# Nesquiko/Latticeum

Hardware: AMD Instinct MI355X
Metric: fold-steps/sec (Ajtai commit+fold) at d=1024 (higher is better)
Workload: dtype u64 (Goldilocks mod-p integer); 1 GPU; configs[2] at d=1024: commit+fold step, X^1024+1, W=16384, kappa=32, K=15; rho is an input; transcript, linearization, sumchecks, Mz outside the step; d=1024, W=16384, N=81920, kappa=32

## Files before the change

include/lf.h:

```cpp
#ifndef LATTICEUM_AMD_LF_H
#define LATTICEUM_AMD_LF_H
#include <stddef.h>
#include <stdint.h>

#ifdef __cplusplus
extern "C" {
#endif

typedef struct lf_ctx lf_ctx;
typedef struct lf_ajtai lf_ajtai;
typedef struct lf_transcript lf_transcript;
typedef struct lf_comm lf_comm;
typedef struct lf_ccs lf_ccs;

enum lf_status {
  LF_OK = 0,
  LF_ERR_INVALID_ARG = 1,
  LF_ERR_UNSUPPORTED_RING = 2,
  LF_ERR_WRONG_WITNESS_LENGTH = 3,
  LF_ERR_WRONG_COMMITMENT_LENGTH = 4,
  LF_ERR_WRONG_AJTAI_DIMENSIONS = 5,
  LF_ERR_DECOMPOSITION_OVERFLOW = 6,
  LF_ERR_INCORRECT_LENGTH = 7,
  LF_ERR_CHALLENGE_BYTES = 8,
// ... 147 lines not shown
int lf_dev_fold_step_sharded(lf_ctx *ctx, const lf_ajtai *aj, const lf_params *pr, size_t W,
                             const lf_fold_step_bufs *b, lf_comm *comm);

int lf_comm_unique_id(uint8_t *id, size_t len);
int lf_comm_init(lf_ctx *ctx, int nranks, int rank, const uint8_t *id, size_t len, lf_comm **out);
int lf_comm_wrap(lf_ctx *ctx, void *nccl_comm, lf_comm **out);
void lf_comm_destroy(lf_comm *comm);
int lf_comm_size(const lf_comm *comm);
int lf_comm_rank(const lf_comm *comm);
int lf_comm_allreduce_modp(lf_ctx *ctx, lf_comm *comm, uint64_t *x, size_t n);
int lf_fold_reduce_allranks(lf_ctx *ctx, lf_comm *comm, uint64_t *cm0, size_t cm0_len, uint64_t *f0,
                            size_t f0_len);

int lf_dev_fold_lcccs(lf_ctx *ctx, int d, int nwit, const uint64_t *rho, const uint64_t *rho_coeff,
                      const uint64_t *eta, size_t t, const uint64_t *xwh, size_t l1, const uint64_t *theta,
                      uint64_t *u0, uint64_t *x0, uint64_t *v0);
int lf_dev_compute_x_s(lf_ctx *ctx, const lf_params *pr, const uint64_t *x, size_t m, uint64_t *x_s);

int lf_dev_poseidon2_permute(lf_ctx *ctx, uint64_t *states, size_t n);
int lf_dev_poseidon2_permute_rounds(lf_ctx *ctx, uint64_t *states, size_t n, int rounds);
int lf_dev_gl_probe(lf_ctx *ctx, int op, const uint64_t *a, const uint64_t *b, int s, int m, uint64_t *out,
                    size_t n);
int lf_ctx_fold_flag(lf_ctx *ctx, int *out);
enum { LF_PLAN_FOLDING = 0, LF_PLAN_LIN = 1, LF_PLAN_LIN_EQ = 2 };
int lf_sumcheck_round_plan(int d, size_t half, int nf, int kind, int out[8]);
int lf_sumcheck_dot_plan(int d, size_t n, int out[4]);
int lf_dev_fill_uniform(lf_ctx *ctx, uint64_t *out, size_t n, uint64_t seed);
int lf_dev_modp_sum(lf_ctx *ctx, const uint64_t *in, int nparts, size_t len, uint64_t *out);

int lf_dev_limb_split(lf_ctx *ctx, const uint64_t *x, size_t n, uint64_t *lo, uint64_t *hi);
int lf_dev_limb_join(lf_ctx *ctx, const uint64_t *lo, const uint64_t *hi, size_t n, uint64_t *out);

enum { LF_COMB_FOLDING = 0, LF_COMB_LINEARIZATION = 1 };
typedef struct {
  int kind;
  int nk, tau, bsmall;
  const uint64_t *mu;
  int q;
  const uint64_t *c;
  const int *S_off;
  const int *S_idx;
} lf_comb;
int lf_dev_eq_table(lf_ctx *ctx, int d, const uint64_t *r, int nv, uint64_t *out);
int lf_dev_get_fhat(lf_ctx *ctx, int d, const uint64_t *f_coeff, size_t N, int nv, uint64_t *out);
int lf_dev_mle_fix_first(lf_ctx *ctx, int d, const uint64_t *in, size_t in_stride, int nm, int nv,
                         const uint64_t *r_base, uint64_t *out, size_t out_stride);
// ... 307 lines not shown
```

latticeum_amd/__init__.py:

```python
from __future__ import annotations

import ctypes as C
from dataclasses import dataclass

import numpy as np

from ._lib import LfComb, LfFoldStepBufs, LfParams, load

P = (1 << 64) - (1 << 32) + 1
REPR_CANONICAL = 0
REPR_MONTGOMERY = 1
SUPPORTED_D = (24, 16, 32, 64, 128, 256, 512, 1024, 2048, 4096)
AJTAI_SEED_POSEIDON2 = 1
AJTAI_SEED_SPLITMIX = 2


class LfError(RuntimeError):
    def __init__(self, code: int, msg: str):
        super().__init__(f"lf error {code}: {msg}")
        self.code = code


def goldilocks_dp(d: int = 24) -> LfParams:
    return load().lf_goldilocks_dp(d)
# ... 59 lines not shown
            self.lib.lf_stream_destroy(st)
        self._masked = []

    def __del__(self):
        try:
            self.close()
        except Exception:
            pass

    def check(self, rc: int):
        if rc != 0:
            msg = self.lib.lf_ctx_last_error(self.h).decode() or self.lib.lf_status_string(rc).decode()
            raise LfError(rc, msg)

    def set_stream(self, hip_stream: int | None):
        self.check(self.lib.lf_ctx_set_stream(self.h, hip_stream))

    def sync(self):
        self.check(self.lib.lf_ctx_sync(self.h))

    def fold_flag(self) -> int:
        out = C.c_int()
        self.check(self.lib.lf_ctx_fold_flag(self.h, C.byref(out)))
        return out.value

    def use_cu_mask(self, cus):
        cus = list(cus)
        st = self.cu_mask_stream(cus)
        self.set_stream(st)
        self.check(self.lib.lf_ctx_set_cu_count(self.h, len(set(cus))))
        return st

    def set_contract_stream(self, hip_stream: int | None):
        self.check(self.lib.lf_ctx_set_contract_stream(self.h, hip_stream))

    def cu_mask_stream(self, cus):
        cus = list(cus)
        words = (max(cus) // 32 + 1) if cus else 1
        mask = (C.c_uint32 * words)()
        for i in cus:
            mask[i // 32] |= 1 << (i % 32)
        st = C.c_void_p()
        rc = self.lib.lf_stream_create_cu_mask(self.device, mask, words, C.byref(st))
        if rc != 0:
            raise LfError(rc, "lf_stream_create_cu_mask")
        self._masked = getattr(self, "_masked", []) + [st.value]
# ... 1162 lines not shown
```

latticeum_amd/_lib.py:

```python
from __future__ import annotations

import ctypes as C
import os
from pathlib import Path

PKG = Path(__file__).resolve().parent
LIB_PATH = PKG / "liblatticeum_amd.so"

SZ, I, U64, VP = C.c_size_t, C.c_int, C.c_uint64, C.c_void_p
U64P = C.POINTER(C.c_uint64)
U8P = C.POINTER(C.c_uint8)


class LfParams(C.Structure):
    _fields_ = [("d", I), ("B", U64), ("L", I), ("b_small", U64), ("K", I)]


class LfFoldStepBufs(C.Structure):
    _fields_ = [
        ("w_ccs", VP), ("acc_cm", VP), ("acc_f_coeff", VP), ("rho", VP),
        ("f_coeff", VP), ("f", VP), ("cm", VP),
        ("fk_coeff", VP * 2), ("fk", VP * 2), ("wk", VP * 2), ("y", VP * 2),
        ("f0", VP), ("f0_coeff", VP), ("w_ccs0", VP), ("cm0", VP), ("planes", VP * 2),
    ]
# ... 93 lines not shown
    "lf_decompose_witness": (I, [VP, C.POINTER(LfParams), VP, SZ, VP, VP, VP, I]),
    "lf_commit": (I, [VP, VP, C.POINTER(LfParams), VP, SZ, SZ, VP, VP, VP, I]),
    "lf_fold_hot": (I, [VP, VP, C.POINTER(LfParams), VP, VP, VP, VP, SZ, VP, VP, VP, VP, VP, VP, I]),
    "lf_short_challenge": (I, [VP, SZ, I, VP]),
    "lf_poseidon2_permute": (I, [VP, VP, SZ]),
    "lf_dev_crt": (I, [VP, VP, SZ, I]),
    "lf_dev_icrt": (I, [VP, VP, SZ, I]),
    "lf_dev_ring_mul": (I, [VP, VP, VP, VP, SZ, I]),
    "lf_dev_to_montgomery": (I, [VP, VP, SZ]),
    "lf_dev_from_montgomery": (I, [VP, VP, SZ]),
    "lf_dev_witness_from_w_ccs": (I, [VP, C.POINTER(LfParams), VP, SZ, VP, VP]),
    "lf_dev_witness_from_f": (I, [VP, C.POINTER(LfParams), VP, SZ, VP, VP]),
    "lf_dev_witness_from_f_coeff": (I, [VP, C.POINTER(LfParams), VP, SZ, VP, VP]),
    "lf_dev_decompose_witness": (I, [VP, C.POINTER(LfParams), VP, SZ, VP, VP, VP]),
    "lf_dev_ajtai_commit": (I, [VP, VP, C.POINTER(VP), I, VP]),
    "lf_dev_commit_y0": (I, [VP, C.POINTER(LfParams), VP, VP, SZ]),
    "lf_dev_fold": (I, [VP, I, VP, C.POINTER(VP), I, SZ, VP]),
    "lf_dev_fold_step": (I, [VP, VP, C.POINTER(LfParams), SZ, C.POINTER(LfFoldStepBufs)]),
    "lf_dev_fold_step_batch": (I, [VP, I, VP, C.POINTER(LfParams), SZ, VP]),
    "lf_dev_poseidon2_permute": (I, [VP, VP, SZ]),
    "lf_dev_poseidon2_permute_rounds": (I, [VP, VP, SZ, I]),
    "lf_dev_gl_probe": (I, [VP, I, VP, VP, I, I, VP, SZ]),
    "lf_ctx_fold_flag": (I, [VP, C.POINTER(I)]),
    "lf_sumcheck_round_plan": (I, [I, SZ, I, I, C.POINTER(I * 8)]),
    "lf_sumcheck_dot_plan": (I, [I, SZ, C.POINTER(I * 4)]),
    "lf_dev_fhat_lincomb_digits": (I, [VP, I, VP, SZ, SZ, I, I, VP, VP]),
    "lf_dev_fill_uniform": (I, [VP, VP, SZ, U64]),
    "lf_dev_modp_sum": (I, [VP, VP, I, SZ, VP]),
    "lf_dev_limb_split": (I, [VP, VP, SZ, VP, VP]),
    "lf_dev_limb_join": (I, [VP, VP, VP, SZ, VP]),
    "lf_transcript_new": (VP, []),
    "lf_transcript_free": (None, [VP]),
    "lf_transcript_observe": (None, [VP, U64]),
    "lf_transcript_sample": (U64, [VP]),
    "lf_transcript_absorb_ring": (None, [VP, VP, SZ, I, I]),
    "lf_transcript_get_challenge": (None, [VP, VP]),
    "lf_transcript_squeeze_bytes": (None, [VP, VP, SZ]),
    "lf_transcript_get_short_challenges": (I, [VP, I, SZ, VP]),
    "lf_hash_iter": (None, [VP, SZ, VP]),
    "lf_hash_iter_nperm": (SZ, [SZ]),
    "lf_hash_iter_states": (I, [VP, SZ, VP, VP, SZ]),
    "lf_acc_comm": (I, [C.POINTER(LfLcccs), I, VP]),
    "lf_ivc_step_comm": (I, [U64, VP, VP, VP, VP, VP]),
    "lf_state_i_comm": (I, [VP, U64, VP, VP, VP, VP]),
    "lf_vm_regs_comm": (I, [VP, SZ, VP]),
    "lf_vm_mem_ops_vec_comm": (I, [VP, U64, C.c_uint32, C.c_uint32, VP]),
# ... 149 lines not shown
```

latticeum_amd/csrc/api_internal.hpp:

```cpp
#pragma once
#include <hip/hip_runtime.h>
#include <rccl/rccl.h>

#include <cstring>
#include <map>
#include <string>
#include <vector>

#include "../../include/lf.h"
#include "gl.hpp"
#include "kernels.hpp"
#include "launch.hpp"

struct Tables {
  uint64_t *mem = nullptr;
  ring::NegaTables fwd{}, inv{};
};

struct TimedLaunch {
  hipEvent_t a, b;
  int nvec;
  int count = 1;
};

// ... 16 lines not shown

struct lf_ctx {
  int device = 0;
  hipStream_t own = nullptr, cur = nullptr;
  int *d_err = nullptr;
  int *d_sync = nullptr;
  std::string last_error;
  std::map<int, Tables> tables;
  uint64_t *scratch = nullptr;
  size_t scratch_elems = 0;
  uint64_t *ybuf = nullptr;
  size_t ybuf_elems = 0;
  uint4 *frag = nullptr;
  size_t frag_elems = 0;
  uint32_t *smg = nullptr;
  size_t smg_elems = 0;
  uint32_t *fkeys = nullptr;
  size_t fkeys_elems = 0;
  uint64_t *faux = nullptr;
  int32_t *fpart = nullptr;
  size_t fpart_elems = 0;
  size_t faux_elems = 0;
  long fold_flag_at = -1;
  uint64_t *sink = nullptr;
  uint8_t *dead = nullptr;
  size_t dead_elems = 0;
  uint4 *zero80 = nullptr;
  uint32_t *toptbl = nullptr;
  StepState step{};
  int ncu = 0;
  uint64_t *stage = nullptr;
  size_t stage_elems = 0;
  uint64_t *limb = nullptr;
  size_t limb_elems = 0;
  uint64_t *tmp = nullptr;
  size_t tmp_elems = 0;
  uint64_t *sc = nullptr;
  size_t sc_elems = 0;
  uint64_t *ptrs = nullptr;
  size_t ptrs_elems = 0;
  int *sel = nullptr;
  size_t sel_elems = 0;
  uint64_t *rel = nullptr;
  size_t rel_elems = 0;
  uint64_t *hmsg = nullptr;
  size_t hmsg_elems = 0;
// ... 181 lines not shown
```

latticeum_amd/csrc/api_step.hip:

```cpp
#include <algorithm>

#include "api_internal.hpp"

namespace {

struct PhaseTimer {
  lf_ctx *c;
  int phase;
  hipEvent_t a = nullptr;
  PhaseTimer(lf_ctx *ctx, int ph) : c(ctx), phase(ph) {
    if (c->timing && hipEventCreate(&a) == hipSuccess) (void)hipEventRecord(a, c->cur);
  }
  ~PhaseTimer() {
    hipEvent_t b = nullptr;
    if (a && hipEventCreate(&b) == hipSuccess) {
      (void)hipEventRecord(b, c->cur);
      c->pending.push_back({a, b, -1 - phase});
    }
  }
};

bool n4k_ok(const Tables *t, int d, int lbs, int K) { return d == 4096 && lbs == 1 && K <= 15 && t->fwd.tw4; }

enum class Decomp { Plain, Fused1024, Fused24, Fused4k, FusedPow2 };
// ... 229 lines not shown
  if (c->timing) c->pending.push_back({ea, eb, nvec});
  return LF_OK;
}

lfk::OutPtrs fold_dst(const lf_params *pr, const lf_fold_step_bufs *b, size_t kd, uint64_t *commit_cm,
                      bool z0 = false) {
  lfk::OutPtrs dst{};
  const int extra = commit_cm ? 1 : 0;
  if (commit_cm) dst.p[0] = z0 ? b->y[1] : commit_cm;
  for (int s = 0; s < 2; s++)
    for (int k = 1; k < pr->K; k++) dst.p[extra + s * (pr->K - 1) + k - 1] = b->y[s] + (size_t)k * kd;
  return dst;
}

int fold_finish(lf_ctx *c, const lf_ajtai *aj, const lf_params *pr, int lb, int lbs, size_t W,
                const lf_fold_step_bufs *b, uint64_t *cm_i, bool cm1_out = false) {
  const int d = pr->d, L = pr->L, K = pr->K, nw = 2 * K;
  const size_t N = W * (size_t)L, kappa = aj->kappa;
  Tables *t;
  LF_TRY(get_tables(c, d, t));
  LF_HIP(c, lfk::y0_cm0(b->acc_cm, cm_i, b->y[0], b->y[1], b->rho, kappa, d, lbs, K, b->cm0, c->cur, cm1_out));
  const StepState &st = c->step;
  c->fold_flag_at = -1;
  auto fk_rows = [&] {
    lfk::VecPtrs fx{};
    for (int s = 0; s < 2; s++)
      for (int k = 0; k < K; k++) fx.p[s * K + k] = b->fk[s] + (size_t)k * N * d;
    return fx;
  };
  switch (st.N == N ? st.path : FoldPath::Ntt) {
    case FoldPath::Coeff1024:
    case FoldPath::Coeff1024Rows: {
      const size_t tab_u64 = ((size_t)nw * lfk::FOLD_RT + 7) / 8, aux = (size_t)nw * 1024 + tab_u64 + 1;
      LF_TRY(grow(c, c->fkeys, c->fkeys_elems, 2 * N * (size_t)K * 64 + 2 * N));
      uint32_t *nz = c->fkeys + 2 * N * (size_t)K * 64;
      LF_TRY(grow(c, c->faux, c->faux_elems, aux));
      uint64_t *rc = c->faux;
      uint8_t *tab = reinterpret_cast<uint8_t *>(c->faux + (size_t)nw * 1024);
      int *bad = reinterpret_cast<int *>(c->faux + aux - 1);
      c->fold_flag_at = (long)(aux - 1);
      {
        PhaseTimer pt(c, LF_PHASE_FOLD);
        for (int s = 0; s < 2; s++)
          LF_HIP(c, lfk::fold_keys(st.smg_side[s], N, K, c->fkeys + (size_t)s * N * K * 64, c->cur, nz + (size_t)s * N));
        LF_HIP(c, lfk::fold_rho_tables(b->rho, nw, rc, tab, bad, t->inv, c->d_sync, c->cur));
        const int ks_n = lfk::fold_coeff_splits(N, K, c->ncu);
        if (ks_n > 1) LF_TRY(grow(c, c->fpart, c->fpart_elems, (size_t)ks_n * N * 1024));
        const bool in_launch = st.path == FoldPath::Coeff1024Rows;
        const lfk::FoldFallback fb{c->frag, aj->geom.nch, aj->geom.Lp, aj->geom.Wp, st.fold_rows, b->rho, b->f0};
        LF_HIP(c, lfk::fold_coeff(c->fkeys, tab, bad, N, K, b->f0_coeff, c->ncu, c->cur,
                                  ks_n > 1 ? c->fpart : nullptr, in_launch ? &fb : nullptr, L, nz));
        if (!in_launch) LF_HIP(c, lfk::fold(b->rho, fk_rows(), nw, N, d, b->f0, c->cur, bad));
      }
      PhaseTimer pt(c, LF_PHASE_FROM_F);
      LF_HIP(c, lfk::from_fcoeff_n32(b->f0_coeff, W, lb, L, b->f0, b->w_ccs0, t->fwd, bad, c->cur, &t->inv));
      return LF_OK;
    }
    case FoldPath::Masks24:
    case FoldPath::Masks24Packed: {
      const uint2 *m0 = st.masks24[0], *m1 = st.masks24[1];
      LF_TRY(grow(c, c->faux, c->faux_elems, (size_t)nw * 13 + 1));
      uint32_t *rc = reinterpret_cast<uint32_t *>(c->faux);
      int *bad = reinterpret_cast<int *>(c->faux + (size_t)nw * 13);
      c->fold_flag_at = (long)nw * 13;
      {
        PhaseTimer pt(c, LF_PHASE_FOLD);
        LF_HIP(c, lfk::fold_phi72_rho(b->rho, nw, rc, bad, c->cur));
        LF_HIP(c, lfk::fold_phi72_coeff(m0, m1, rc, bad, N, K, L, lb, b->f0_coeff, b->f0, b->w_ccs0, c->cur));
        if (st.path == FoldPath::Masks24Packed)
          LF_HIP(c, lfk::fold_phi72_masks(m0, m1, b->rho, K, N, b->f0, bad, c->cur));
        else
          LF_HIP(c, lfk::fold(b->rho, fk_rows(), nw, N, d, b->f0, c->cur, bad));
      }
      PhaseTimer pt(c, LF_PHASE_FROM_F);
// ... 356 lines not shown
```

latticeum_amd/csrc/fold_coeff.hip:

```cpp
#include "digitpack.hpp"
#include "digits.hpp"
#include "frag.hpp"
#include "kernels.hpp"
#include "launch.hpp"
#include "ntt32.hpp"

namespace lfk {

namespace {
constexpr int FD = 1024;
constexpr int FC_KEYROW = 64;

__device__ __forceinline__ uint32_t spread8(uint32_t x) {
  x &= 0xFFu;
  x = (x | (x << 12)) & 0x000F000Fu;
  x = (x | (x << 6)) & 0x03030303u;
  x = (x | (x << 3)) & 0x11111111u;
  return x;
}

__global__ void __launch_bounds__(256) k_pack_keys(const uint32_t *smg, size_t ncol, int K, uint32_t *keys,
                                                   uint32_t *nz) {
  const size_t t = blockIdx.x * (size_t)blockDim.x + threadIdx.x;
  if (t >= (ncol * 16 + 63) / 64 * 64) return;
// ... 40 lines not shown
      lo[4 * qd + i] = L;
      hi[4 * qd + i] = H;
    }
  uint4 *dst = reinterpret_cast<uint4 *>(keys + col * K * FC_KEYROW + 32 * h + q0);
  for (int k = 0; k < K; k++) {
    uint32_t o[4];
#pragma unroll
    for (int qd = 0; qd < 4; qd++) {
      uint32_t x = 0;
#pragma unroll
      for (int i = 0; i < 4; i++) {
        const int u = 4 * qd + i;
        const uint32_t nib = (k < 8 ? lo[u] >> (4 * k) : hi[u] >> (4 * (k - 8))) & 0xFu;
        x |= (nib | ((hi[u] >> 28) << 4)) << (8 * i);
      }
      o[qd] = x;
    }
    dst[k * (FC_KEYROW / 4)] = make_uint4(o[0], o[1], o[2], o[3]);
  }
}

constexpr int RP_WAVES = 2;
__global__ void __launch_bounds__(64 * RP_WAVES) k_rho_prep(const uint64_t *rho, int nw, uint64_t *rc, uint8_t *tab,
                                                           int *bad, const uint64_t *mid_ig, int *sync) {
  __shared__ uint64_t lds_all[RP_WAVES * n32::WAVE_U64];
  __shared__ uint64_t mid[n32::MID_U64];
  __shared__ int any;
  n32::stage_mid(mid, mid_ig);
  if (threadIdx.x == 0) any = 0;
  __syncthreads();
  const int lane = threadIdx.x & 63, wib = threadIdx.x >> 6, r = lane & 31, h = lane >> 5;
  uint64_t *T = lds_all + wib * n32::WAVE_U64 + h * n32::HALF_U64;
  bool out = false;
  for (int i0 = 2 * RP_WAVES * blockIdx.x; i0 < nw; i0 += 2 * RP_WAVES * gridDim.x) {
    const int i = i0 + 2 * wib + h;
    const bool ok = i < nw;
    uint64_t v[32];
    n32::load_row32(rho + (size_t)(ok ? i : 0) * FD + r, v);
    n32::inverse(v, mid, T, r);
    if (ok) {
      uint64_t *rci = rc + (size_t)i * FD + r;
      uint8_t *ti = tab + (size_t)i * FOLD_RT;
#pragma unroll
      for (int k = 0; k < 32; k++) {
        const int c = r + 32 * k;
        const int64_t sv = signed_rep(v[k]);
        out |= sv > 127 || sv < -127;
        rci[32 * k] = v[k];
        ti[1024 - c] = (uint8_t)(int8_t)sv;
        if (c > 0) ti[2048 - c] = (uint8_t)(int8_t)(-sv);
      }
      for (int o = 2048 + r; o < FOLD_RT; o += 32) ti[o] = 0;
      if (r == 0) ti[0] = 0;
    }
  }
  if (out) any = 1;
  __syncthreads();
  if (threadIdx.x == 0) {
    if (any) atomicOr(&sync[0], 1);
    __threadfence();
    if (atomicAdd(&sync[1], 1) == (int)gridDim.x - 1) {
      *bad = atomicExch(&sync[0], 0);
      atomicExch(&sync[1], 0);
    }
  }
}

__device__ __forceinline__ v4i tile_a(const uint8_t *ri, int o, int sh) {
  const uint32_t *p = reinterpret_cast<const uint32_t *>(ri + (o & ~3));
  const uint32_t d0 = p[0], d1 = p[1], d2 = p[2], d3 = p[3], d4 = p[4];
  v4i a;
  a[0] = (int)__builtin_amdgcn_alignbyte(d1, d0, sh);
  a[1] = (int)__builtin_amdgcn_alignbyte(d2, d1, sh);
  a[2] = (int)__builtin_amdgcn_alignbyte(d3, d2, sh);
  a[3] = (int)__builtin_amdgcn_alignbyte(d4, d3, sh);
  return a;
}

constexpr int FC_MAXW = 30;
__global__ void __launch_bounds__(256, 2) k_fold_coeff(const uint32_t *keys, const uint8_t *tab_g, const int *bad,
                                                      size_t N, int K, uint64_t *f0c, int ks_n, int32_t *part,
                                                      FoldFallback fb, int L, const uint32_t *nz) {
  __shared__ __attribute__((aligned(16))) uint8_t rt[FC_MAXW * FOLD_RT];
  __shared__ uint32_t lut[256];
  static_assert(FC_MAXW * FOLD_RT >= 512 * 9 * 8, "fold_frag_block's LDS fits the rho tables'");
  if (*bad) {
    if (fb.frag) {
      const size_t nvb = (size_t)(FD / 16) * fb.nch;
      for (size_t vb = blockIdx.x; vb < nvb; vb += gridDim.x)
        fold_frag_block(vb, fb.frag, fb.nch, fb.Lp, fb.Wp, fb.fr, fb.rho, FD, N, fb.f0,
                        reinterpret_cast<uint64_t *>(rt));
    }
    return;
  }
  const int nw = 2 * K, tid = threadIdx.x;
  for (int x = tid; x < nw * FOLD_RT / 16; x += blockDim.x)
    reinterpret_cast<uint4 *>(rt)[x] = reinterpret_cast<const uint4 *>(tab_g)[x];
  {
    const uint32_t m = tid & 15, s = tid >> 4;
    uint32_t v = 0;
#pragma unroll
    for (int i = 0; i < 4; i++)
      if ((m >> i) & 1) v |= ((s >> i) & 1 ? 0xFFu : 0x01u) << (8 * i);
    lut[tid] = v;
  }
  __syncthreads();
  const int lane = tid & 63, wv = tid >> 6, col = lane & 31, h = lane >> 5;
  const int sh = (-col) & 3;
  const int obase = 1024 + 16 * h - col;
  const size_t W = N / L, ntl = (W + 31) / 32, ntile = ntl * L;
  for (size_t task = blockIdx.x; task < ntile * ks_n; task += gridDim.x) {
    const size_t tile = task / ks_n;
    const int ks = (int)(task % ks_n), iq0 = 4 * (ks * nw / ks_n), iq1 = 4 * ((ks + 1) * nw / ks_n);
    const size_t grp = (tile % ntl) * 32 + col;
    const bool valid = grp < W;
    const size_t e = grp * L + tile / ntl, ee = valid ? e : 0;
    uint32_t live = nz ? (valid ? nz[ee] | (nz[N + ee] << K) : 0u) : 0xFFFFFFFFu;
// ... 52 lines not shown
    }
    if (valid && ks_n > 1) {
      int32_t *out = part + ((size_t)ks * N + e) * FD + 256 * wv + 4 * h;
#pragma unroll
      for (int tt = 0; tt < 8; tt++)
#pragma unroll
        for (int g = 0; g < 4; g++)
          *reinterpret_cast<v4i *>(out + 32 * tt + 8 * g) =
              (v4i){acc[tt][4 * g], acc[tt][4 * g + 1], acc[tt][4 * g + 2], acc[tt][4 * g + 3]};
    } else if (valid) {
      uint64_t *out = f0c + e * FD + 256 * wv + 4 * h;
      auto fe = [](int x) { return x < 0 ? (uint64_t)(int64_t)x + gl::P : (uint64_t)x; };
#pragma unroll
      for (int tt = 0; tt < 8; tt++)
#pragma unroll
        for (int g = 0; g < 4; g++) {
          ulonglong2 *o = reinterpret_cast<ulonglong2 *>(out + 32 * tt + 8 * g);
          o[0] = make_ulonglong2(fe(acc[tt][4 * g]), fe(acc[tt][4 * g + 1]));
          o[1] = make_ulonglong2(fe(acc[tt][4 * g + 2]), fe(acc[tt][4 * g + 3]));
        }
    }
  }
}
__global__ void k_fold_coeff_sum(const int32_t *part, int ks_n, size_t n, const int *bad, uint64_t *f0c) {
  if (*bad) return;
  const size_t q = blockIdx.x * (size_t)blockDim.x + threadIdx.x;
  if (q >= n / 4) return;
  v4i s = *reinterpret_cast<const v4i *>(part + 4 * q);
  for (int k = 1; k < ks_n; k++) s += *reinterpret_cast<const v4i *>(part + (size_t)k * n + 4 * q);
  auto fe = [](int x) { return x < 0 ? (uint64_t)(int64_t)x + gl::P : (uint64_t)x; };
  ulonglong2 *o = reinterpret_cast<ulonglong2 *>(f0c + 4 * q);
  o[0] = make_ulonglong2(fe(s[0]), fe(s[1]));
  o[1] = make_ulonglong2(fe(s[2]), fe(s[3]));
}
}

int fold_coeff_splits(size_t N, int K, int ncu) {
  const size_t ntile = (N + 31) / 32, cap = 2 * (size_t)ncu;
  int best = 1;
  for (int ks = 2; ks <= 2 * K; ks++)
    if ((2 * K) % ks == 0 && ntile * ks <= cap) best = ks;
  return best;
}

hipError_t fold_keys(const uint32_t *smg, size_t ncol, int K, uint32_t *keys, hipStream_t st, uint32_t *nz) {
  if (K < 1 || K > 15) return hipErrorInvalidValue;
  if (!ncol) return hipSuccess;
  hipLaunchKernelGGL(k_pack_keys, dim3(blocks(ncol * 16, 256)), dim3(256), 0, st, smg, ncol, K, keys,
                     nz);
  return hipGetLastError();
}

hipError_t fold_rho_tables(const uint64_t *rho, int nw, uint64_t *rc, uint8_t *tab, int *bad,
                           const ring::NegaTables &inv, int *sync, hipStream_t st) {
  if (nw < 1 || nw > FC_MAXW || !inv.mid || !sync) return hipErrorInvalidValue;
  const int per = 2 * RP_WAVES;
  hipLaunchKernelGGL(k_rho_prep, dim3((nw + per - 1) / per), dim3(64 * RP_WAVES), 0, st, rho, nw, rc, tab, bad,
                     inv.mid, sync);
  return hipGetLastError();
}

hipError_t fold_coeff(const uint32_t *keys, const uint8_t *tab, const int *bad, size_t N, int K, uint64_t *f0c,
                      int ncu, hipStream_t st, int32_t *part, const FoldFallback *fb, int L, const uint32_t *nz) {
  FoldFallback fbv{};
  if (fb) fbv = *fb;
  if (K < 1 || 2 * K > FC_MAXW || ncu < 1 || L < 1 || N % L) return hipErrorInvalidValue;
  if (!N) return hipSuccess;
  const int ks_n = part ? fold_coeff_splits(N, K, ncu) : 1;
  const size_t ntile = (N / L + 31) / 32 * L;
  const size_t ntask = ntile * ks_n, cap = 2 * (size_t)ncu;
  hipLaunchKernelGGL(k_fold_coeff, dim3((unsigned)(ntask < cap ? ntask : cap)), dim3(256), 0, st, keys, tab, bad, N,
                     K, f0c, ks_n, part, fbv, L, nz);
  if (ks_n > 1) {
    const size_t n = N * FD;
    hipLaunchKernelGGL(k_fold_coeff_sum, dim3(blocks(n / 4, 256)), dim3(256), 0, st, part, ks_n, n, bad,
                       f0c);
  }
  return hipGetLastError();
}

}
```

latticeum_amd/csrc/kernels.hpp:

```cpp
#pragma once
#include <hip/hip_runtime.h>
#include <stddef.h>
#include <stdint.h>

#include "digitpack.hpp"
#include "fragpos.hpp"
#include "ring.hpp"

#define LF_MAX_VECS 32
#define LF_MAX_KTILES 4
#define LF_MAX_STEPS 8

namespace lfk {

struct VecPtrs {
  const uint64_t *p[LF_MAX_VECS];
};
struct OutPtrs {
  uint64_t *p[LF_MAX_VECS];
};

struct DeadUnits {
  const uint8_t *flags = nullptr;
  uint32_t rows = 0;
// ... 97 lines not shown
  int nside;
  int row_p0[2] = {-1, -1};
  uint2 *masks[2] = {nullptr, nullptr};
  uint32_t *smg[2] = {nullptr, nullptr};
  uint8_t *dead = nullptr;
  int prepacked = 0;
};
struct FoldRows {
  int row[LF_MAX_VECS];
  int rho[LF_MAX_VECS];
  int n;
  DeadUnits dead;
};
hipError_t fold_frag(const uint4 *frag, const FragGeom &g, const FoldRows &fr, const uint64_t *rho, int d, size_t N,
                     uint64_t *out, hipStream_t st, const int *run_if = nullptr);
hipError_t decompose_fused(const FusedSides &sd, size_t N, int lb, int L, int K, const ring::NegaTables &fwd, uint4 *frag, int nch, int *err, uint64_t *sink, int ncu,
                           hipStream_t st);

hipError_t decompose_pow2(const FusedSides &sd, size_t N, int d, int lb, int L, int K, const ring::NegaTables &fwd,
                          uint4 *frag, int nch, int *err, hipStream_t st);
hipError_t expand_smp2(const uint32_t *smg, size_t N, int d, int K, uint64_t *fck, hipStream_t st);

constexpr int FOLD_RT = 2080;
hipError_t fold_keys(const uint32_t *smg, size_t ncol, int K, uint32_t *keys, hipStream_t st, uint32_t *nz = nullptr);
hipError_t fold_rho_tables(const uint64_t *rho, int nw, uint64_t *rc, uint8_t *tab, int *bad,
                           const ring::NegaTables &inv, int *sync, hipStream_t st);
int fold_coeff_splits(size_t N, int K, int ncu);
struct FoldFallback {
  const uint4 *frag;
  int nch, Lp;
  size_t Wp;
  FoldRows fr;
  const uint64_t *rho;
  uint64_t *f0;
};
hipError_t fold_coeff(const uint32_t *keys, const uint8_t *tab, const int *bad, size_t N, int K, uint64_t *f0c,
                      int ncu, hipStream_t st, int32_t *part = nullptr, const FoldFallback *fb = nullptr, int L = 1,
                      const uint32_t *nz = nullptr);
hipError_t from_fcoeff_n32(uint64_t *f_coeff, size_t W, int lb, int L, uint64_t *f, uint64_t *w_ccs,
                           const ring::NegaTables &fwd, const int *gate, hipStream_t st,
                           const ring::NegaTables *inv = nullptr);

hipError_t decompose_phi72_sides(const FusedSides &sd, size_t N, int lb, int L, int lbs, int K, int *err,
                                 uint4 *frag, int nch, hipStream_t st, bool *masks_written = nullptr,
                                 bool *dead_written = nullptr);
hipError_t fold_phi72_rho(const uint64_t *rho, int nw, uint32_t *rc, int *bad, hipStream_t st);
hipError_t fold_phi72_coeff(const uint2 *masks0, const uint2 *masks1, const uint32_t *rc, const int *bad, size_t N,
                            int K, int L, int lb, uint64_t *f0_coeff, uint64_t *f0, uint64_t *w_ccs0, hipStream_t st);
hipError_t fold_phi72_masks(const uint2 *masks0, const uint2 *masks1, const uint64_t *rho, int K, size_t N,
                            uint64_t *f0, const int *run_if, hipStream_t st);
hipError_t expand_phi72(const uint2 *planes, size_t n, uint64_t *fc, uint64_t *f, hipStream_t st);
hipError_t expand_sm(const uint32_t *smg, size_t N, int K, uint64_t *fck, hipStream_t st);
hipError_t expand_sm8(const uint32_t *sm8, size_t N, int K, uint64_t *fck, hipStream_t st);
hipError_t decompose_n4k(const FusedSides &sd, size_t N, int lb, int L, int K, uint64_t *sm4,
                         const ring::NegaTables &fwd, int *err, uint64_t *sink, int ncu, hipStream_t st,
                         uint4 *frag = nullptr, int nch = 0);

hipError_t from_f_n4k(const uint64_t *f, size_t W, int lb, int L, uint64_t *f_coeff, uint64_t *w_ccs,
                      const ring::NegaTables &inv, hipStream_t st);
hipError_t from_w_ccs_n4k(const uint64_t *w_ccs, size_t W, int lb, int L, uint64_t *f_coeff, uint64_t *f,
                          const ring::NegaTables &fwd, const ring::NegaTables &inv, int *err, hipStream_t st);
// ... 143 lines not shown
```

latticeum_amd/csrc/lf_api.hip:

```cpp
#include <dlfcn.h>

#include <cstdio>
#include <algorithm>
#include <memory>

#include "ajtai_seed.hpp"
#include "api_internal.hpp"

int get_tables(lf_ctx *c, int d, Tables *&out) {
  auto it = c->tables.find(d);
  if (it != c->tables.end()) {
    out = &it->second;
    return LF_OK;
  }
  Tables t;
  if (d != 24) {
    const size_t extra = d == 1024 ? 2048 : d == 4096 ? 2048 + 2 * 4096 + 1024 : 0;
    const size_t az_off = 4 * (size_t)d + extra;
    std::vector<uint64_t> h(az_off + (d == 1024 ? 1024 : d == 4096 ? 4 * 4096 + 4 * 1024 : 0));
    const uint64_t psi = gl::pow(7, (gl::P - 1) / (2 * (uint64_t)d));
    const uint64_t psi_inv = gl::inv(psi), w = gl::mul(psi, psi), w_inv = gl::mul(psi_inv, psi_inv);
    const uint64_t dinv = gl::inv((uint64_t)d);
    uint64_t a = 1, b = 1, x = dinv, y = 1;
    for (int j = 0; j < d; j++) {
// ... 379 lines not shown
  if (!c) return LF_ERR_INVALID_ARG;
  LF_HIP(c, hipStreamSynchronize(c->cur));
  int e = 0;
  LF_HIP(c, hipMemcpy(&e, c->d_err, sizeof(int), hipMemcpyDeviceToHost));
  if (e) {
    LF_HIP(c, hipMemset(c->d_err, 0, sizeof(int)));
    return fail(c, LF_ERR_DECOMPOSITION_OVERFLOW, "a coefficient needed more digits than padding_size");
  }
  return LF_OK;
}

int lf_ctx_fold_flag(lf_ctx *c, int *out) {
  DevGuard g(c);
  if (!c || !out) return LF_ERR_INVALID_ARG;
  LF_HIP(c, hipStreamSynchronize(c->cur));
  *out = -1;
  if (c->fold_flag_at < 0 || !c->faux || (size_t)c->fold_flag_at >= c->faux_elems) return LF_OK;
  int bad = 0;
  LF_HIP(c, hipMemcpy(&bad, c->faux + c->fold_flag_at, sizeof(int), hipMemcpyDeviceToHost));
  *out = bad ? 1 : 0;
  return LF_OK;
}

int lf_ctx_reserve(lf_ctx *c, size_t kappa, size_t ncols, int d, int nvec) {
  DevGuard g(c);
  if (!c || !ring_ok(d) || nvec < 1 || nvec > LF_MAX_VECS) return LF_ERR_INVALID_ARG;
  Tables *t;
  LF_TRY(get_tables(c, d, t));
  lf_ajtai probe;
  probe.kappa = kappa;
  probe.ncols = ncols;
  probe.d = d;
  if (use_mfma(d, kappa)) {
    probe.Af = reinterpret_cast<uint4 *>(1);
    probe.geom = ajtai_geom(ncols);
    probe.geom.qperm = d == 4096;
    LF_TRY(grow(c, c->frag, c->frag_elems, lfk::frag_elems(probe.geom, d)));
  }
  LF_TRY(grow(c, c->scratch, c->scratch_elems, partial_elems(&probe, nvec)));
  return grow(c, c->ybuf, c->ybuf_elems, (size_t)nvec * kappa * d);
}

int lf_ctx_kernel_timing(lf_ctx *c, int enable) {
  DevGuard g(c);
  if (!c) return LF_ERR_INVALID_ARG;
  LF_TRY(drain_timing(c));
// ... 603 lines not shown
```

Baseline: 62.53 fold-steps/s.

## Add one-level Karatsuba split for coefficient-domain fold via int8 MFMA

```diff
diff --git a/include/lf.h b/include/lf.h
--- a/include/lf.h
+++ b/include/lf.h
@@ -193,6 +193,7 @@
 int lf_dev_gl_probe(lf_ctx *ctx, int op, const uint64_t *a, const uint64_t *b, int s, int m, uint64_t *out,
                     size_t n);
 int lf_ctx_fold_flag(lf_ctx *ctx, int *out);
+int lf_ctx_fold_level(lf_ctx *ctx, int *out);
 enum { LF_PLAN_FOLDING = 0, LF_PLAN_LIN = 1, LF_PLAN_LIN_EQ = 2 };
 int lf_sumcheck_round_plan(int d, size_t half, int nf, int kind, int out[8]);
 int lf_sumcheck_dot_plan(int d, size_t n, int out[4]);
diff --git a/latticeum_amd/__init__.py b/latticeum_amd/__init__.py
--- a/latticeum_amd/__init__.py
+++ b/latticeum_amd/__init__.py
@@ -105,6 +105,11 @@
     def fold_flag(self) -> int:
         out = C.c_int()
         self.check(self.lib.lf_ctx_fold_flag(self.h, C.byref(out)))
+        return out.value
+
+    def fold_level(self) -> int:
+        out = C.c_int()
+        self.check(self.lib.lf_ctx_fold_level(self.h, C.byref(out)))
         return out.value
 
     def use_cu_mask(self, cus):
diff --git a/latticeum_amd/_lib.py b/latticeum_amd/_lib.py
--- a/latticeum_amd/_lib.py
+++ b/latticeum_amd/_lib.py
@@ -139,6 +139,7 @@
     "lf_dev_poseidon2_permute_rounds": (I, [VP, VP, SZ, I]),
     "lf_dev_gl_probe": (I, [VP, I, VP, VP, I, I, VP, SZ]),
     "lf_ctx_fold_flag": (I, [VP, C.POINTER(I)]),
+    "lf_ctx_fold_level": (I, [VP, C.POINTER(I)]),
     "lf_sumcheck_round_plan": (I, [I, SZ, I, I, C.POINTER(I * 8)]),
     "lf_sumcheck_dot_plan": (I, [I, SZ, C.POINTER(I * 4)]),
     "lf_dev_fhat_lincomb_digits": (I, [VP, I, VP, SZ, SZ, I, I, VP, VP]),
diff --git a/latticeum_amd/csrc/api_internal.hpp b/latticeum_amd/csrc/api_internal.hpp
--- a/latticeum_amd/csrc/api_internal.hpp
+++ b/latticeum_amd/csrc/api_internal.hpp
@@ -62,6 +62,7 @@
   size_t fpart_elems = 0;
   size_t faux_elems = 0;
   long fold_flag_at = -1;
+  bool fold_has_level = false;
   uint64_t *sink = nullptr;
   uint8_t *dead = nullptr;
   size_t dead_elems = 0;
diff --git a/latticeum_amd/csrc/api_step.hip b/latticeum_amd/csrc/api_step.hip
--- a/latticeum_amd/csrc/api_step.hip
+++ b/latticeum_amd/csrc/api_step.hip
@@ -275,6 +275,7 @@
   LF_HIP(c, lfk::y0_cm0(b->acc_cm, cm_i, b->y[0], b->y[1], b->rho, kappa, d, lbs, K, b->cm0, c->cur, cm1_out));
   const StepState &st = c->step;
   c->fold_flag_at = -1;
+  c->fold_has_level = false;
   auto fk_rows = [&] {
     lfk::VecPtrs fx{};
     for (int s = 0; s < 2; s++)
@@ -284,7 +285,8 @@
   switch (st.N == N ? st.path : FoldPath::Ntt) {
     case FoldPath::Coeff1024:
     case FoldPath::Coeff1024Rows: {
-      const size_t tab_u64 = ((size_t)nw * lfk::FOLD_RT + 7) / 8, aux = (size_t)nw * 1024 + tab_u64 + 1;
+      const size_t tab_u64 = (lfk::fold_tab_bytes(nw) + 7) / 8, aux = (size_t)nw * 1024 + tab_u64 + 1;
+      const int kara = lfk::fold_kara_cap();
       LF_TRY(grow(c, c->fkeys, c->fkeys_elems, 2 * N * (size_t)K * 64 + 2 * N));
       uint32_t *nz = c->fkeys + 2 * N * (size_t)K * 64;
       LF_TRY(grow(c, c->faux, c->faux_elems, aux));
@@ -292,17 +294,18 @@
       uint8_t *tab = reinterpret_cast<uint8_t *>(c->faux + (size_t)nw * 1024);
       int *bad = reinterpret_cast<int *>(c->faux + aux - 1);
       c->fold_flag_at = (long)(aux - 1);
+      c->fold_has_level = true;
       {
         PhaseTimer pt(c, LF_PHASE_FOLD);
         for (int s = 0; s < 2; s++)
           LF_HIP(c, lfk::fold_keys(st.smg_side[s], N, K, c->fkeys + (size_t)s * N * K * 64, c->cur, nz + (size_t)s * N));
-        LF_HIP(c, lfk::fold_rho_tables(b->rho, nw, rc, tab, bad, t->inv, c->d_sync, c->cur));
+        LF_HIP(c, lfk::fold_rho_tables(b->rho, nw, rc, tab, bad, t->inv, c->d_sync, c->cur, kara));
         const int ks_n = lfk::fold_coeff_splits(N, K, c->ncu);
         if (ks_n > 1) LF_TRY(grow(c, c->fpart, c->fpart_elems, (size_t)ks_n * N * 1024));
         const bool in_launch = st.path == FoldPath::Coeff1024Rows;
         const lfk::FoldFallback fb{c->frag, aj->geom.nch, aj->geom.Lp, aj->geom.Wp, st.fold_rows, b->rho, b->f0};
         LF_HIP(c, lfk::fold_coeff(c->fkeys, tab, bad, N, K, b->f0_coeff, c->ncu, c->cur,
-                                  ks_n > 1 ? c->fpart : nullptr, in_launch ? &fb : nullptr, L, nz));
+                                  ks_n > 1 ? c->fpart : nullptr, in_launch ? &fb : nullptr, L, nz, kara));
         if (!in_launch) LF_HIP(c, lfk::fold(b->rho, fk_rows(), nw, N, d, b->f0, c->cur, bad));
       }
       PhaseTimer pt(c, LF_PHASE_FROM_F);
diff --git a/latticeum_amd/csrc/fold_coeff.hip b/latticeum_amd/csrc/fold_coeff.hip
--- a/latticeum_amd/csrc/fold_coeff.hip
+++ b/latticeum_amd/csrc/fold_coeff.hip
@@ -86,7 +86,7 @@
 
 constexpr int RP_WAVES = 2;
 __global__ void __launch_bounds__(64 * RP_WAVES) k_rho_prep(const uint64_t *rho, int nw, uint64_t *rc, uint8_t *tab,
-                                                           int *bad, const uint64_t *mid_ig, int *sync) {
+                                                           int *bad, const uint64_t *mid_ig, int *sync, int kara_cap) {
   __shared__ uint64_t lds_all[RP_WAVES * n32::WAVE_U64];
   __shared__ uint64_t mid[n32::MID_U64];
   __shared__ int any;
@@ -96,6 +96,8 @@
   const int lane = threadIdx.x & 63, wib = threadIdx.x >> 6, r = lane & 31, h = lane >> 5;
   uint64_t *T = lds_all + wib * n32::WAVE_U64 + h * n32::HALF_U64;
   bool out = false;
+  int64_t hi1 = 0, lo1 = 0;
+  uint8_t *tab1 = tab + (size_t)nw * FOLD_RT;
   for (int i0 = 2 * RP_WAVES * blockIdx.x; i0 < nw; i0 += 2 * RP_WAVES * gridDim.x) {
     const int i = i0 + 2 * wib + h;
     const bool ok = i < nw;
@@ -116,15 +118,38 @@
       }
       for (int o = 2048 + r; o < FOLD_RT; o += 32) ti[o] = 0;
       if (r == 0) ti[0] = 0;
-    }
-  }
-  if (out) any = 1;
+      if (kara_cap >= 1) {
+        uint8_t *t1 = tab1 + (size_t)i * 3 * FOLD_RT1;
+#pragma unroll
+        for (int k = 0; k < 16; k++) {
+          const int c = r + 32 * k;
+          const int64_t a = signed_rep(v[k]), b = signed_rep(v[k + 16]);
+          const int64_t g[2][3] = {{a, b - a, a + b}, {-b, a + b, a - b}};
+#pragma unroll
+          for (int p = 0; p < 3; p++) {
+            const int64_t g1 = c > 0 ? g[1][p] : 0;
+            hi1 = max(hi1, max(g[0][p], g1));
+            lo1 = min(lo1, min(g[0][p], g1));
+            t1[p * FOLD_RT1 + 512 - c] = (uint8_t)(int8_t)g[0][p];
+            if (c > 0) t1[p * FOLD_RT1 + 1024 - c] = (uint8_t)(int8_t)g[1][p];
+          }
+        }
+        if (r < FOLD_RT1 - 1024 + 1)
+#pragma unroll
+          for (int p = 0; p < 3; p++) t1[p * FOLD_RT1 + (r ? 1023 + r : 0)] = 0;
+      }
+    }
+  }
+  const bool out1 = hi1 > 127 || lo1 < -128;
+  if (out || out1) atomicOr(&any, (out ? 1 : 0) | (out1 ? 2 : 0));
   __syncthreads();
   if (threadIdx.x == 0) {
-    if (any) atomicOr(&sync[0], 1);
+    if (any) atomicOr(&sync[0], any);
     __threadfence();
     if (atomicAdd(&sync[1], 1) == (int)gridDim.x - 1) {
-      *bad = atomicExch(&sync[0], 0);
+      const int f = atomicExch(&sync[0], 0);
+      bad[0] = f & 1;
+      bad[1] = f ? 0 : kara_cap;
       atomicExch(&sync[1], 0);
     }
   }
@@ -157,6 +182,7 @@
     }
     return;
   }
+  if (bad[1] != 0) return;
   const int nw = 2 * K, tid = threadIdx.x;
   for (int x = tid; x < nw * FOLD_RT / 16; x += blockDim.x)
     reinterpret_cast<uint4 *>(rt)[x] = reinterpret_cast<const uint4 *>(tab_g)[x];
@@ -255,6 +281,191 @@
     }
   }
 }
+constexpr int FC1_TAB = 3 * FOLD_RT1;
+
+__device__ __forceinline__ uint32_t add_bytes(uint32_t a, uint32_t b) {
+  return ((a & 0x7F7F7F7Fu) + (b & 0x7F7F7F7Fu)) ^ ((a ^ b) & 0x80808080u);
+}
+
+template <int MODE>
+__device__ __forceinline__ void kara1_pass(v16i (&acc)[8], const uint8_t *tp, const uint32_t *lut,
+                                           const uint32_t *kb0, size_t side1, int K, uint32_t live, int i0,
+                                           int i1, int rh, int obase, int sh) {
+  constexpr int NV = MODE == 0 ? 2 : 1;
+  auto next_live = [&](int i) {
+    while (i < i1 && !((live >> i) & 1u)) i++;
+    return i;
+  };
+  auto krow = [&](int i) {
+    const int s = i >= K;
+    return reinterpret_cast<const uint4 *>(kb0 + ((s ? side1 : 0) + (i - s * K) * FC_KEYROW + (MODE == 2 ? 16 : 0)));
+  };
+  int i = next_live(i0);
+  if (i >= i1) return;
+  uint4 kq[NV][4];
+  auto load_keys = [&](int pl, int m) {
+    const uint4 *p = krow(pl);
+#pragma unroll
+    for (int v = 0; v < NV; v++) kq[v][m] = p[4 * v + m];
+  };
+  auto key = [&](int v, int q) {
+    const uint4 &u = kq[v][q >> 2];
+    return (q & 3) == 0 ? u.x : (q & 3) == 1 ? u.y : (q & 3) == 2 ? u.z : u.w;
+  };
+  auto fetch_a = [&](const uint8_t *r, int dl, uint32_t (&d)[5]) {
+    const int o = obase - 32 * dl;
+    const uint32_t *p = reinterpret_cast<const uint32_t *>(r + (o & ~3));
+#pragma unroll
+    for (int x = 0; x < 5; x++) d[x] = p[x];
+  };
+  auto asm_a = [&](const uint32_t (&d)[5], v4i &a) {
+#pragma unroll
+    for (int x = 0; x < 4; x++) a[x] = (int)__builtin_amdgcn_alignbyte(d[x + 1], d[x], sh);
+  };
+  uint32_t rl[NV][4];
+  auto fetch_b = [&](int q, int j0) {
+#pragma unroll
+    for (int v = 0; v < NV; v++)
+#pragma unroll
+      for (int j = j0; j < j0 + 2; j++) rl[v][j] = lut[(key(v, q) >> (8 * j)) & 0xFF];
+  };
+  auto asm_b = [&](int x0, v4i &b) {
+#pragma unroll
+    for (int x = x0; x < x0 + 2; x++) b[x] = (int)(MODE == 0 ? add_bytes(rl[0][x], rl[NV - 1][x]) : rl[0][x]);
+  };
+#pragma unroll
+  for (int m = 0; m < 4; m++) load_keys(i, m);
+  int nx = next_live(i + 1);
+  const uint8_t *ri = tp + i * FC1_TAB;
+  v4i A[8], An[8], bb[2];
+  uint32_t rd[5], wd[5];
+  {
+    uint32_t d[7][5];
+#pragma unroll
+    for (int tt = 1; tt < 8; tt++) fetch_a(ri, 8 * rh + tt, d[tt - 1]);
+#pragma unroll
+    for (int tt = 1; tt < 8; tt++) asm_a(d[tt - 1], A[tt]);
+  }
+  fetch_b(0, 0);
+  fetch_b(0, 2);
+  asm_b(0, bb[0]);
+  asm_b(2, bb[0]);
+  fetch_a(ri, 8 * rh, rd);
+  fetch_b(1, 0);
+  fetch_b(1, 2);
+  for (;;) {
+    const bool more = nx < i1;
+    const int pn = more ? nx : i;
+    const uint8_t *rin = tp + pn * FC1_TAB;
+#pragma unroll
+    for (int q = 0; q < 16; q++) {
+#pragma unroll
+      for (int k = 0; k < 8; k++) {
+        const int tt = (k + 1) & 7;
+        __builtin_amdgcn_sched_barrier(0);
+        acc[tt] = __builtin_amdgcn_mfma_i32_32x32x32_i8(A[(tt - q) & 7], bb[q & 1], acc[tt], 0, 0, 0);
+        __builtin_amdgcn_sched_barrier(0);
+        if (k == 0) asm_a(rd, A[(16 - q) & 7]);
+        if (k == 1) asm_b(0, bb[(q + 1) & 1]);
+        if (k == 2) asm_b(2, bb[(q + 1) & 1]);
+        if (k == 3) fetch_a(q < 15 ? ri : rin, 8 * rh - ((q + 1) & 15), rd);
+        if (k == 4) fetch_b((q + 2) & 15, 0);
+        if (k == 5) fetch_b((q + 2) & 15, 2);
+        if (k == 6) {
+          if (q >= 8 && q <= 14) asm_a(wd, An[q - 7]);
+          if (q >= 7 && q <= 13) fetch_a(rin, 8 * rh + q - 6, wd);
+        }
+        if (k == 7 && (q & 3) == 2) load_keys(pn, q >> 2);
+      }
+      __builtin_amdgcn_sched_barrier(0);
+    }
+    if (!more) break;
+#pragma unroll
+    for (int tt = 1; tt < 8; tt++) A[tt] = An[tt];
+    i = nx;
+    ri = rin;
+    nx = next_live(i + 1);
+  }
+}
+
+__global__ void __launch_bounds__(256, 1) k_fold_coeff_kara1(const uint32_t *keys, const uint8_t *tab1_g,
+                                                            const int *bad, size_t N, int K, uint64_t *f0c, int ks_n,
+                                                            int32_t *part, int L, const uint32_t *nz) {
+  __shared__ __attribute__((aligned(16))) uint8_t rt[FC_MAXW * FC1_TAB];
+  __shared__ uint32_t lut[256];
+  if (bad[1] != 1) return;
+  const int nw = 2 * K, tid = threadIdx.x;
+  for (int x = tid; x < nw * FC1_TAB / 16; x += blockDim.x)
+    reinterpret_cast<uint4 *>(rt)[x] = reinterpret_cast<const uint4 *>(tab1_g)[x];
+  {
+    const uint32_t m = tid & 15, s = tid >> 4;
+    uint32_t v = 0;
+#pragma unroll
+    for (int i = 0; i < 4; i++)
+      if ((m >> i) & 1) v |= ((s >> i) & 1 ? 0xFFu : 0x01u) << (8 * i);
+    lut[tid] = v;
+  }
+  __syncthreads();
+  const int lane = tid & 63, wv = tid >> 6, col = lane & 31, h = lane >> 5;
+  const int sh = (-col) & 3, rh = wv & 1;
+  const int obase = 512 + 16 * h - col;
+  const size_t W = N / L, ntl = (W + 31) / 32, ntile = ntl * L, npair = (ntile + 1) / 2;
+  for (size_t task = blockIdx.x; task < npair * ks_n; task += gridDim.x) {
+    const size_t tile = 2 * (task / ks_n) + (wv >> 1);
+    if (tile >= ntile) continue;
+    const int ks = (int)(task % ks_n), i0 = ks * nw / ks_n, i1 = (ks + 1) * nw / ks_n;
+    const size_t grp = (tile % ntl) * 32 + col;
+    const bool valid = grp < W;
+    const size_t e = grp * L + tile / ntl, ee = valid ? e : 0;
+    uint32_t live = nz ? (valid ? nz[ee] | (nz[N + ee] << K) : 0u) : 0xFFFFFFFFu;
+#pragma unroll
+    for (int o = 1; o < 32; o <<= 1) live |= __shfl_xor(live, o);
+    live = __builtin_amdgcn_readfirstlane(live);
+    const uint32_t *kb0 = keys + ee * K * FC_KEYROW + 32 * h;
+    const size_t side1 = N * K * FC_KEYROW;
+    v16i a0[8], a1[8];
+#pragma unroll
+    for (int tt = 0; tt < 8; tt++)
+#pragma unroll
+      for (int i = 0; i < 16; i++) a0[tt][i] = 0;
+    kara1_pass<0>(a0, rt, lut, kb0, side1, K, live, i0, i1, rh, obase, sh);
+#pragma unroll
+    for (int tt = 0; tt < 8; tt++) {
+      a1[tt] = a0[tt];
+      a0[tt] = -a0[tt];
+    }
+    auto store = [&](const v16i (&a)[8], int row) {
+      if (!valid) return;
+      if (ks_n > 1) {
+        int32_t *out = part + ((size_t)ks * N + e) * FD + row;
+#pragma unroll
+        for (int tt = 0; tt < 8; tt++)
+#pragma unroll
+          for (int g = 0; g < 4; g++)
+            *reinterpret_cast<v4i *>(out + 32 * tt + 8 * g) =
+                (v4i){a[tt][4 * g], a[tt][4 * g + 1], a[tt][4 * g + 2], a[tt][4 * g + 3]};
+      } else {
+        uint64_t *out = f0c + e * FD + row;
+        auto fe = [](int x) { return x < 0 ? (uint64_t)(int64_t)x + gl::P : (uint64_t)x; };
+#pragma unroll
+        for (int tt = 0; tt < 8; tt++)
+#pragma unroll
+          for (int g = 0; g < 4; g++) {
+            ulonglong2 *o = reinterpret_cast<ulonglong2 *>(out + 32 * tt + 8 * g);
+            o[0] = make_ulonglong2(fe(a[tt][4 * g]), fe(a[tt][4 * g + 1]));
+            o[1] = make_ulonglong2(fe(a[tt][4 * g + 2]), fe(a[tt][4 * g + 3]));
+          }
+      }
+    };
+    kara1_pass<2>(a0, rt + 2 * FOLD_RT1, lut, kb0, side1, K, live, i0, i1, rh, obase, sh);
+#pragma unroll
+    for (int tt = 0; tt < 8; tt++) a0[tt] = -a0[tt];
+    store(a0, 256 * rh + 4 * h);
+    kara1_pass<1>(a1, rt + FOLD_RT1, lut, kb0, side1, K, live, i0, i1, rh, obase, sh);
+    store(a1, 512 + 256 * rh + 4 * h);
+  }
+}
+
 __global__ void k_fold_coeff_sum(const int32_t *part, int ks_n, size_t n, const int *bad, uint64_t *f0c) {
   if (*bad) return;
   const size_t q = blockIdx.x * (size_t)blockDim.x + threadIdx.x;
@@ -276,6 +487,12 @@
   return best;
 }
 
+int fold_kara_cap() {
+  const char *e = getenv("LATTICEUM_AMD_FOLD_KARA");
+  if (!e || e[0] < '0' || e[0] > '0' + FOLD_KARA_MAX || e[1]) return FOLD_KARA_MAX;
+  return e[0] - '0';
+}
+
 hipError_t fold_keys(const uint32_t *smg, size_t ncol, int K, uint32_t *keys, hipStream_t st, uint32_t *nz) {
   if (K < 1 || K > 15) return hipErrorInvalidValue;
   if (!ncol) return hipSuccess;
@@ -285,16 +502,18 @@
 }
 
 hipError_t fold_rho_tables(const uint64_t *rho, int nw, uint64_t *rc, uint8_t *tab, int *bad,
-                           const ring::NegaTables &inv, int *sync, hipStream_t st) {
-  if (nw < 1 || nw > FC_MAXW || !inv.mid || !sync) return hipErrorInvalidValue;
+                           const ring::NegaTables &inv, int *sync, hipStream_t st, int kara_cap) {
+  if (nw < 1 || nw > FC_MAXW || !inv.mid || !sync || kara_cap < 0 || kara_cap > FOLD_KARA_MAX)
+    return hipErrorInvalidValue;
   const int per = 2 * RP_WAVES;
   hipLaunchKernelGGL(k_rho_prep, dim3((nw + per - 1) / per), dim3(64 * RP_WAVES), 0, st, rho, nw, rc, tab, bad,
-                     inv.mid, sync);
+                     inv.mid, sync, kara_cap);
   return hipGetLastError();
 }
 
 hipError_t fold_coeff(const uint32_t *keys, const uint8_t *tab, const int *bad, size_t N, int K, uint64_t *f0c,
-                      int ncu, hipStream_t st, int32_t *part, const FoldFallback *fb, int L, const uint32_t *nz) {
+                      int ncu, hipStream_t st, int32_t *part, const FoldFallback *fb, int L, const uint32_t *nz,
+                      int kara_cap) {
   FoldFallback fbv{};
   if (fb) fbv = *fb;
   if (K < 1 || 2 * K > FC_MAXW || ncu < 1 || L < 1 || N % L) return hipErrorInvalidValue;
@@ -304,6 +523,11 @@
   const size_t ntask = ntile * ks_n, cap = 2 * (size_t)ncu;
   hipLaunchKernelGGL(k_fold_coeff, dim3((unsigned)(ntask < cap ? ntask : cap)), dim3(256), 0, st, keys, tab, bad, N,
                      K, f0c, ks_n, part, fbv, L, nz);
+  if (kara_cap >= 1) {
+    const size_t ntask1 = (ntile + 1) / 2 * ks_n;
+    hipLaunchKernelGGL(k_fold_coeff_kara1, dim3((unsigned)(ntask1 < (size_t)ncu ? ntask1 : (size_t)ncu)), dim3(256),
+                       0, st, keys, tab + (size_t)2 * K * FOLD_RT, bad, N, K, f0c, ks_n, part, L, nz);
+  }
   if (ks_n > 1) {
     const size_t n = N * FD;
     hipLaunchKernelGGL(k_fold_coeff_sum, dim3(blocks(n / 4, 256)), dim3(256), 0, st, part, ks_n, n, bad,
diff --git a/latticeum_amd/csrc/kernels.hpp b/latticeum_amd/csrc/kernels.hpp
--- a/latticeum_amd/csrc/kernels.hpp
+++ b/latticeum_amd/csrc/kernels.hpp
@@ -143,9 +143,13 @@
 hipError_t expand_smp2(const uint32_t *smg, size_t N, int d, int K, uint64_t *fck, hipStream_t st);
 
 constexpr int FOLD_RT = 2080;
+constexpr int FOLD_RT1 = 1040;
+constexpr int FOLD_KARA_MAX = 1;
+constexpr size_t fold_tab_bytes(int nw) { return (size_t)nw * (FOLD_RT + 3 * FOLD_RT1); }
+int fold_kara_cap();
 hipError_t fold_keys(const uint32_t *smg, size_t ncol, int K, uint32_t *keys, hipStream_t st, uint32_t *nz = nullptr);
 hipError_t fold_rho_tables(const uint64_t *rho, int nw, uint64_t *rc, uint8_t *tab, int *bad,
-                           const ring::NegaTables &inv, int *sync, hipStream_t st);
+                           const ring::NegaTables &inv, int *sync, hipStream_t st, int kara_cap = 0);
 int fold_coeff_splits(size_t N, int K, int ncu);
 struct FoldFallback {
   const uint4 *frag;
@@ -157,7 +161,7 @@
 };
 hipError_t fold_coeff(const uint32_t *keys, const uint8_t *tab, const int *bad, size_t N, int K, uint64_t *f0c,
                       int ncu, hipStream_t st, int32_t *part = nullptr, const FoldFallback *fb = nullptr, int L = 1,
-                      const uint32_t *nz = nullptr);
+                      const uint32_t *nz = nullptr, int kara_cap = 0);
 hipError_t from_fcoeff_n32(uint64_t *f_coeff, size_t W, int lb, int L, uint64_t *f, uint64_t *w_ccs,
                            const ring::NegaTables &fwd, const int *gate, hipStream_t st,
                            const ring::NegaTables *inv = nullptr);
diff --git a/latticeum_amd/csrc/lf_api.hip b/latticeum_amd/csrc/lf_api.hip
--- a/latticeum_amd/csrc/lf_api.hip
+++ b/latticeum_amd/csrc/lf_api.hip
@@ -425,6 +425,18 @@
   return LF_OK;
 }
 
+int lf_ctx_fold_level(lf_ctx *c, int *out) {
+  DevGuard g(c);
+  if (!c || !out) return LF_ERR_INVALID_ARG;
+  LF_HIP(c, hipStreamSynchronize(c->cur));
+  *out = -1;
+  if (!c->fold_has_level || c->fold_flag_at < 0 || !c->faux || (size_t)c->fold_flag_at >= c->faux_elems) return LF_OK;
+  int w[2] = {0, 0};
+  LF_HIP(c, hipMemcpy(w, c->faux + c->fold_flag_at, sizeof w, hipMemcpyDeviceToHost));
+  *out = w[1];
+  return LF_OK;
+}
+
 int lf_ctx_reserve(lf_ctx *c, size_t kappa, size_t ncols, int d, int nvec) {
   DevGuard g(c);
   if (!c || !ring_ok(d) || nvec < 1 || nvec > LF_MAX_VECS) return LF_ERR_INVALID_ARG;
```

New measurement: 63.42 fold-steps/s (median of 6 runs). +1.4%, better.
